# grossmanlev/FL-distributed-delay

Measured on AMD Instinct MI355X. Metric: simulated worker-steps/sec (node) @1024 workers, delay 50; aggregation HBM GB/s, higher is better.
Workload: dtype f32

## Files before the change

### fl-distributed-delay_amd/csrc/gemm_direct.h

```cpp
#pragma once
#include "loaders.h"

namespace flsim {

#ifndef FLSIM_DIRECT_FENCES
#define FLSIM_DIRECT_FENCES 1
#endif
constexpr bool DIRECT_FENCES = FLSIM_DIRECT_FENCES;

template <int IH, int IW, int CI, int PAD, int FM, bool WIN = false, int OHX = 0,
          class SRC = BufSrc>
struct Im2colDirect {
    using Unit = typename SRC::Unit;
    static constexpr int PIX = SRC::SM ? GK : CI;
    static constexpr int SLICE = SRC::SM ? IH * IW * GK : GK;
    static constexpr int OH = OHX > 0 ? OHX : IH + 2 * PAD - 2;
    static constexpr int OW = OHX > 0 ? OHX : IW + 2 * PAD - 2;
    static constexpr int PH = OH / 2, PW = OW / 2;
    static constexpr int ROWS_PER_IMG = WIN ? 4 * PH * PW : OH * OW;
    static_assert(CI % 16 == 0, "direct A needs whole 16-channel slices");

    const float* X;
    const float* XL = nullptr;
    int M;
    unsigned vb[FM];
    unsigned short tapmask[FM];
    SRC buf;

    __device__ void setup(int r0, int lane) {
        const int q = lane >> 4;
        buf.init(X, XL, (unsigned long)((M + ROWS_PER_IMG - 1) / ROWS_PER_IMG) * IH * IW * CI * 4);
#pragma unroll
        for (int f = 0; f < FM; ++f) {
            const int m = r0 + 16 * f + (lane & 15);
            long base = 0;
            int msk = 0;
            if (m < M) {
                const int nimg = m / ROWS_PER_IMG;
                const int rem = m - nimg * ROWS_PER_IMG;
                int oh, ow;
                if constexpr (WIN) {
                    const int qq = rem >> 2;
                    const int ph = qq / PW;
                    oh = 2 * ph + ((rem >> 1) & 1);
                    ow = 2 * (qq - ph * PW) + (rem & 1);
                } else {
                    oh = rem / OW;
                    ow = rem - oh * OW;
                }
                base = (long)nimg * IH * IW * CI + ((long)(oh - PAD) * IW + (ow - PAD)) * PIX +
                       4 * q;
#pragma unroll
                for (int t = 0; t < 9; ++t) {
                    const int ih = oh + t / 3 - PAD, iw = ow + t % 3 - PAD;
                    if ((unsigned)ih < (unsigned)IH && (unsigned)iw < (unsigned)IW) msk |= 1 << t;
                }
            }
            vb[f] = (unsigned)base * 4u;
            tapmask[f] = (unsigned short)msk;
        }
    }
    __device__ void load(int ks, Unit (&r)[FM]) const {
        const int cs = ks / 9;
        const int khkw = ks - 9 * cs;
        const int kh = khkw / 3;
        const unsigned off = (unsigned)(((kh * IW + (khkw - 3 * kh)) * PIX + cs * SLICE) * 4);
#pragma unroll
        for (int f = 0; f < FM; ++f) r[f] = buf.ld_or0(vb[f] + off, (tapmask[f] >> khkw) & 1);
    }
};

template <int TR, int NT>
struct RowsKCStage {
    static constexpr int ROWS = TR;
    static constexpr bool KC = true;
    static constexpr int TOTAL = ROWS * 4;
    static constexpr int UNITS = (TOTAL + NT - 1) / NT;
    static constexpr int FLOATS = KCTile<ROWS>::FLOATS + 4;
    const float* P;
    long ld;
    int NR;
    unsigned rowb[UNITS];
    int dst[UNITS];
    BufSrc buf;
    __device__ void setup(int r0, int tid) {
        buf.init(P, (unsigned long)NR * ld * 4);
#pragma unroll
        for (int j = 0; j < UNITS; ++j) {
            const int u0 = tid + j * NT;
            const bool real = u0 < TOTAL;
            const int u = real ? u0 : u0 % TOTAL;
            const int r = u >> 2, q = u & 3;
            rowb[j] = r0 + r < NR ? (unsigned)(((long)(r0 + r) * ld + 4 * q) * 4) : BUF_OOB;
            dst[j] = real ? KCTile<ROWS>::chunk_off(r, q) : KCTile<ROWS>::FLOATS;
        }
    }
    __device__ void load(int ks, f32x4 (&r)[UNITS]) const {
#pragma unroll
        for (int j = 0; j < UNITS; ++j)
            r[j] = buf.ld(rowb[j] == BUF_OOB ? BUF_OOB : rowb[j] + (unsigned)(ks * GK * 4));
    }
    __device__ void store(float* lds, const f32x4 (&r)[UNITS]) const {
#pragma unroll
        for (int j = 0; j < UNITS; ++j) *reinterpret_cast<f32x4*>(lds + dst[j]) = r[j];
    }
};

template <int FM, int FN, int WAVES, int KB, int DEPTH, class AD, class BL, class EPI>
__global__ void __launch_bounds__(64 * WAVES)
gemm_direct_kernel(AD ad, BL bl, EPI epi, int ksteps, int tiles_m, int tiles_n) {
    constexpr int BM = 16 * FM * WAVES;
    constexpr int BN = 16 * FN;
    static_assert(BL::ROWS == BN && BL::KC, "B loader: k-contiguous tile of BN rows");
    constexpr int BFL = BL::FLOATS;
    constexpr int STG = KB * BFL;
    constexpr bool STAGED = IsStaged<EPI>::value;
    constexpr int STAGE_LD = BN + 4;
    constexpr int BASE_FL = 2 * STG;
    constexpr int WROWS = 16 * FM;
    constexpr int WM_FIT = (BASE_FL > 8192 ? BASE_FL : 8192) / (WROWS * STAGE_LD);
    constexpr int WM_PASS = WM_FIT < 1 ? 1 : (WM_FIT > WAVES ? WAVES : WM_FIT);
    constexpr int LDS_FL = STAGED && WM_PASS * WROWS * STAGE_LD > BASE_FL
                               ? WM_PASS * WROWS * STAGE_LD : BASE_FL;
    __shared__ __attribute__((aligned(16))) float lds[LDS_FL];

    const int tid = threadIdx.x;
    const int lane = tid & 63;
    const int wave = tid >> 6;
    const int nb = gridDim.x;
    const int b = blockIdx.x;
    const int q = nb / 8, r = nb % 8, xcd = b % 8;
    const int L = (xcd < r ? xcd * (q + 1) : r * (q + 1) + (xcd - r) * q) + b / 8;
    const int tn = L % tiles_n;
    const int tm = L / tiles_n;
    const int m0 = tm * BM;
    const int n0 = tn * BN;

    ad.setup(m0 + wave * WROWS, lane);
    bl.setup(n0, tid);

    f32x4 acc[FM][FN];
#pragma unroll
    for (int i = 0; i < FM; ++i)
#pragma unroll
        for (int j = 0; j < FN; ++j) acc[i][j] = f32x4{0.f, 0.f, 0.f, 0.f};

    constexpr int R = DEPTH + 1;
    static_assert(KB % R == 0, "the A register ring index must be static");
    f32x4 ra[R][FM];
    f32x4 rb[BL::UNITS];
    const int nst = ksteps / KB;
#pragma unroll
    for (int d = 0; d < DEPTH; ++d) ad.load(d, ra[d]);
#pragma unroll
    for (int kk = 0; kk < KB; ++kk) {
        bl.load(kk, rb);
        bl.store(lds + kk * BFL, rb);
    }
    __syncthreads();
    if constexpr (WAVES == 8) {
        if (wave >= 4) __builtin_amdgcn_s_setprio(1);
    }
    for (int s = 0; s < nst; ++s) {
        const float* Bs = lds + (s & 1) * STG;
        float* Bn = lds + ((s + 1) & 1) * STG;
        const int kn = (s + 1) * KB;
#pragma unroll
        for (int kk = 0; kk < KB; ++kk) {
            const int ks = s * KB + kk;
            if (kk > 0) bl.store(Bn + (kk - 1) * BFL, rb);
            bl.load(kn + kk, rb);
            ad.load(ks + DEPTH, ra[(kk + DEPTH) % R]);
            if constexpr (DIRECT_FENCES) __builtin_amdgcn_sched_barrier(0);
            f32x4 bf[FN];
#pragma unroll
            for (int j = 0; j < FN; ++j) bf[j] = read_frag<true, BN>(Bs + kk * BFL, 16 * j, lane);
#pragma unroll
            for (int kq = 0; kq < 4; ++kq)
#pragma unroll
                for (int i = 0; i < FM; ++i)
#pragma unroll
                    for (int j = 0; j < FN; ++j)
                        acc[i][j] = mfma16(ra[kk % R][i][kq], bf[j][kq], acc[i][j]);
            if constexpr (DIRECT_FENCES) __builtin_amdgcn_sched_barrier(0);
        }
        bl.store(Bn + (KB - 1) * BFL, rb);
        __syncthreads();
    }

    if constexpr (STAGED) {
        static_assert(BN == EPI::NCOL || (IsPartial<EPI>::value && EPI::NCOL % BN == 0),
                      "staged epilogue needs the full row in one block");
        constexpr int PASSES = (WAVES + WM_PASS - 1) / WM_PASS;
#pragma unroll 1
        for (int pass = 0; pass < PASSES; ++pass) {
            __syncthreads();
            if (wave / WM_PASS == pass) {
#pragma unroll
                for (int i = 0; i < FM; ++i)
#pragma unroll
                    for (int j = 0; j < FN; ++j) {
                        const int ml = (wave - pass * WM_PASS) * WROWS + 16 * i + 4 * (lane >> 4);
                        const int nl = 16 * j + (lane & 15);
#pragma unroll
                        for (int rr = 0; rr < 4; ++rr)
                            lds[(ml + rr) * STAGE_LD + nl] = epi.value(nl, acc[i][j][rr]);
                    }
            }
            __syncthreads();
            const int w_hi = (pass + 1) * WM_PASS < WAVES ? (pass + 1) * WM_PASS : WAVES;
            staged_store(epi, lds, STAGE_LD, m0 + pass * WM_PASS * WROWS,
                         (w_hi - pass * WM_PASS) * WROWS, n0, BN, tid, 64 * WAVES);
        }
    } else {
#pragma unroll
        for (int i = 0; i < FM; ++i)
#pragma unroll
            for (int j = 0; j < FN; ++j) {
                const int m = m0 + wave * WROWS + 16 * i + 4 * (lane >> 4);
                const int n = n0 + 16 * j + (lane & 15);
                epi.apply4(m, n, 0, acc[i][j]);
            }
    }
}
// ... 3 lines not shown
```

### fl-distributed-delay_amd/csrc/gemm_dx6.h

```cpp
#pragma once
#include "gemm_direct.h"
#include "gemm_x6.h"

namespace flsim {

#ifndef FLSIM_DX6_FENCES
#define FLSIM_DX6_FENCES 1
#endif
constexpr bool DX6_FENCES = FLSIM_DX6_FENCES;

template <int TR, int NT, int NPL>
struct RowsKCStageXs {
    using Unit = XsUnit;
    static constexpr int ROWS = TR;
    static constexpr bool KC = true;
    static constexpr int TOTAL = ROWS * 4;
    static constexpr int UNITS = (TOTAL + NT - 1) / NT;
    static constexpr int PLANE = KCTile<ROWS>::FLOATS;
    static constexpr int SPARE = NPL * PLANE;
    static constexpr int FLOATS = NPL * PLANE + 4;
    static_assert(NPL == 2 || NPL == 3, "");
    const float* P;
    const float* PL;
    long ld;
    int NR;
    unsigned rowb[UNITS];
    int dst[UNITS];
    XsSrc buf;
    __device__ void setup(int r0, int tid) {
        buf.init(P, PL, (unsigned long)NR * ld * 4);
#pragma unroll
        for (int j = 0; j < UNITS; ++j) {
            const int u0 = tid + j * NT;
            const bool real = u0 < TOTAL;
            const int u = real ? u0 : u0 % TOTAL;
            const int r = u >> 2, q = u & 3;
            rowb[j] = r0 + r < NR ? (unsigned)(((long)(r0 + r) * ld + 4 * q) * 4) : BUF_OOB;
            dst[j] = real ? KCTile<ROWS>::chunk_off(r, q) : -1;
        }
    }
    __device__ void load(int ks, Unit (&r)[UNITS]) const {
#pragma unroll
        for (int j = 0; j < UNITS; ++j)
            r[j] = buf.ld(rowb[j] == BUF_OOB ? BUF_OOB : rowb[j] + (unsigned)(ks * GK * 4));
    }
    __device__ void store(float* lds, const Unit (&r)[UNITS]) const {
#pragma unroll
        for (int j = 0; j < UNITS; ++j) {
            const bool real = TOTAL % NT == 0 || dst[j] >= 0;
            *reinterpret_cast<f32x4*>(lds + (real ? dst[j] : SPARE)) = r[j].hm;
            *reinterpret_cast<f32x4*>(lds + (real ? dst[j] + PLANE : SPARE)) = xs_lh(r[j]);
            if constexpr (NPL == 3)
                *reinterpret_cast<f32x4*>(lds + (real ? dst[j] + 2 * PLANE : SPARE)) =
                    f32x4{r[j].hm.z, r[j].hm.w, r[j].hm.x, r[j].hm.y};
        }
    }
};

template <int FM, int FN, int WAVES, int KB, int DEPTH, class AD, class BL, class EPI>
__global__ void __launch_bounds__(64 * WAVES)
gemm_dx6_kernel(AD ad, BL bl, EPI epi, int ksteps, int tiles_m, int tiles_n) {
    constexpr int BM = 16 * FM * WAVES;
    constexpr int BN = 16 * FN;
    static_assert(BL::ROWS == BN && BL::KC, "B loader: k-contiguous tile of BN rows");
    constexpr int BFL = BL::FLOATS;
    constexpr int PLANE = BL::PLANE;
    constexpr int STG = KB * BFL;
    constexpr bool STAGED = IsStaged<EPI>::value;
    constexpr int STAGE_LD = BN + 4;
    constexpr int BASE_FL = 2 * STG;
    constexpr int WROWS = 16 * FM;
    constexpr int WM_FIT = (BASE_FL > 8192 ? BASE_FL : 8192) / (WROWS * STAGE_LD);
    constexpr int WM_PASS = WM_FIT < 1 ? 1 : (WM_FIT > WAVES ? WAVES : WM_FIT);
    constexpr int LDS_FL = STAGED && WM_PASS * WROWS * STAGE_LD > BASE_FL
                               ? WM_PASS * WROWS * STAGE_LD : BASE_FL;
    static_assert(LDS_FL * 4 <= 160 * 1024, "LDS");
    __shared__ __attribute__((aligned(16))) float lds[LDS_FL];

    const int tid = threadIdx.x;
    const int lane = tid & 63;
    const int wave = tid >> 6;
    const int nb = gridDim.x;
    const int b = blockIdx.x;
    const int q = nb / 8, r = nb % 8, xcd = b % 8;
    const int L = (xcd < r ? xcd * (q + 1) : r * (q + 1) + (xcd - r) * q) + b / 8;
    const int tn = L % tiles_n;
    const int tm = L / tiles_n;
    const int m0 = tm * BM;
    const int n0 = tn * BN;

    ad.setup(m0 + wave * WROWS, lane);
    bl.setup(n0, tid);

    f32x4 acc[FM][FN];
#pragma unroll
    for (int i = 0; i < FM; ++i)
#pragma unroll
        for (int j = 0; j < FN; ++j) acc[i][j] = f32x4{0.f, 0.f, 0.f, 0.f};

    constexpr int R = DEPTH + 1;
    static_assert(KB % R == 0, "the A register ring index must be static");
    XsUnit ra[R][FM];
    typename BL::Unit rb[BL::UNITS];
    const int nst = ksteps / KB;
#pragma unroll
    for (int d = 0; d < DEPTH; ++d) ad.load(d, ra[d]);
#pragma unroll
    for (int kk = 0; kk < KB; ++kk) {
        bl.load(kk, rb);
        bl.store(lds + kk * BFL, rb);
    }
    __syncthreads();
    if constexpr (WAVES == 8) {
        if (wave >= 4) __builtin_amdgcn_s_setprio(1);
    }
    for (int s = 0; s < nst; ++s) {
        const float* Bs = lds + (s & 1) * STG;
        float* Bn = lds + ((s + 1) & 1) * STG;
        const int kn = (s + 1) * KB;
#pragma unroll
        for (int kk = 0; kk < KB; ++kk) {
            const int ks = s * KB + kk;
            if (kk > 0) bl.store(Bn + (kk - 1) * BFL, rb);
            bl.load(kn + kk, rb);
            ad.load(ks + DEPTH, ra[(kk + DEPTH) % R]);
            if constexpr (DX6_FENCES) __builtin_amdgcn_sched_barrier(0);
            const float* Bk = Bs + kk * BFL;
            f32x4 a0[FM], a1[FM];
#pragma unroll
            for (int i = 0; i < FM; ++i) {
                a0[i] = ra[kk % R][i].hm;
                a1[i] = xs_hl(ra[kk % R][i]);
            }
#pragma unroll
            for (int j = 0; j < FN; ++j) {
                const f32x4 x0 = read_frag<true, BN>(Bk, 16 * j, lane);
                const f32x4 x2 = read_frag<true, BN>(Bk + PLANE, 16 * j, lane);
                f32x4 x1;
                if constexpr (BFL >= 3 * PLANE)
                    x1 = read_frag<true, BN>(Bk + 2 * PLANE, 16 * j, lane);
                else
                    x1 = f32x4{x0.z, x0.w, x0.x, x0.y};
#pragma unroll
                for (int i = 0; i < FM; ++i) {
                    acc[i][j] = x6_step<x6_fresh(true)>(acc[i][j], a0[i], a1[i], x0, x1, x2);
                }
            }
            if constexpr (DX6_FENCES) __builtin_amdgcn_sched_barrier(0);
        }
        bl.store(Bn + (KB - 1) * BFL, rb);
        __syncthreads();
    }

    if constexpr (STAGED) {
        static_assert(BN == EPI::NCOL || (IsPartial<EPI>::value && EPI::NCOL % BN == 0),
                      "staged epilogue needs the full row in one block");
        constexpr int PASSES = (WAVES + WM_PASS - 1) / WM_PASS;
#pragma unroll 1
        for (int pass = 0; pass < PASSES; ++pass) {
            __syncthreads();
            if (wave / WM_PASS == pass) {
#pragma unroll
                for (int i = 0; i < FM; ++i)
#pragma unroll
                    for (int j = 0; j < FN; ++j) {
                        const int ml = (wave - pass * WM_PASS) * WROWS + 16 * i + 4 * (lane >> 4);
                        const int nl = 16 * j + (lane & 15);
#pragma unroll
                        for (int rr = 0; rr < 4; ++rr)
                            lds[(ml + rr) * STAGE_LD + nl] = epi.value(nl, acc[i][j][rr]);
                    }
            }
            __syncthreads();
            const int w_hi = (pass + 1) * WM_PASS < WAVES ? (pass + 1) * WM_PASS : WAVES;
            staged_store(epi, lds, STAGE_LD, m0 + pass * WM_PASS * WROWS,
                         (w_hi - pass * WM_PASS) * WROWS, n0, BN, tid, 64 * WAVES);
        }
    } else {
#pragma unroll
        for (int i = 0; i < FM; ++i)
#pragma unroll
            for (int j = 0; j < FN; ++j) {
                const int m = m0 + wave * WROWS + 16 * i + 4 * (lane >> 4);
                const int n = n0 + 16 * j + (lane & 15);
                epi.apply4(m, n, 0, acc[i][j]);
            }
    }
}

}
```

### fl-distributed-delay_amd/csrc/net_kernels.h

```cpp
#pragma once
#include "epi_xs.h"
#include "gemm_direct.h"
#include "gemm_dx6.h"
#include "gemm_x6.h"
#include "loaders.h"
#include "pn1.h"
#include "probe.h"

namespace flsim {

static __global__ void __launch_bounds__(256)
k_fill_batch(const uint8_t* __restrict__ pool, const int32_t* __restrict__ labels,
             const int32_t* __restrict__ list_a, int len_a, const int32_t* __restrict__ list_b,
             int len_b, const WorkerRec* __restrict__ workers, int n_workers_total, uint64_t seed,
             const float* __restrict__ lut, float* __restrict__ x0, int32_t* __restrict__ y) {
    const int s = blockIdx.x;
    const int w = s / SAMPLES_PER_WORKER;
    const int j = s - w * SAMPLES_PER_WORKER;
    const WorkerRec wr = workers[w];
    const uint32_t bsz = wr.pad ? wr.pad : (uint32_t)SAMPLES_PER_WORKER;
    const uint32_t q = (wr.i >> 20) * SAMPLES_PER_WORKER + (uint32_t)j;
    float* out = x0 + (long)s * 4096;
    if (q >= bsz) {
        if (threadIdx.x == 0) y[s] = -1;
// ... 690 lines not shown
    }
    if (kmin <= 0) return Z;
    int z = (ksteps + kmin - 1) / kmin;
    const int zb = (1024 + tiles - 1) / tiles;
    if (z < zb) z = zb;
    static int fill = -1;
    if (fill < 0) {
        const char* e = lab_env("FLSIM_WSPLIT_FILL");
        fill = e ? atoi(e) : 0;
    }
    if (fill && cap > 0 && z < Z) {
        const long rounds = ((long)tiles * z + cap - 1) / cap;
        const long zf = rounds * cap / tiles;
        if (zf > z) z = (int)(zf < ksteps ? zf : ksteps);
    }
    return z < Z ? z : Z;
}

static int resident_blocks(const void* f, int nt) {
    static int cus = 0;
    if (!cus) {
        int dev = 0;
        if (hipGetDevice(&dev) != hipSuccess ||
            hipDeviceGetAttribute(&cus, hipDeviceAttributeMultiprocessorCount, dev) != hipSuccess)
            cus = -1;
    }
    int per = 0;
    if (cus <= 0 || hipOccupancyMaxActiveBlocksPerMultiprocessor(&per, f, nt, 0) != hipSuccess)
        return 0;
    return per * cus;
}

template <int IH, int IW, int CI, int PAD, int FM, int FN, int WM, int WN, class EPI, int OHX = 0,
          bool X6 = false>
static int conv_like(const float* X, int S, const float* Wpk, int N, int KP, const EPI& epi,
                     hipStream_t st, int kid, int kreal) {
    constexpr int NT = 64 * WM * WN;
    constexpr int BM = 16 * FM * WM, BN = 16 * FN * WN;
    using AL = Im2colKC<IH, IW, CI, PAD, BM, NT, false, OHX>;
    using BL = RowsKC<BN, NT>;
    AL al;
    al.X = X;
    al.M = S * AL::OH * AL::OW;
    BL bl;
    bl.P = Wpk;
    bl.ld = KP;
    bl.NR = N;
    return launch_gemm<FM, FN, WM, WN, X6>(al, bl, epi, al.M, N, KP / GK, 1, st, kid,
                                           2.0 * al.M * N * kreal);
}

template <int IH, int IW, int CI, int PAD, int FM, int FN, int WM, int WN, int OHX = 0, class EPI>
static int conv_x6(const float* X, int S, const float* Wpk, int N, int KP, const EPI& epi,
                   hipStream_t st, int kid, int kreal) {
    return conv_like<IH, IW, CI, PAD, FM, FN, WM, WN, EPI, OHX, true>(X, S, Wpk, N, KP, epi, st,
                                                                      kid, kreal);
}

template <int IH, int IW, int CI, int PAD, int FM, int FMS, int FN, int WM, int WN, class EPI>
static int conv_like_sz(const float* X, int S, const float* Wpk, int N, int KP, const EPI& epi,
                        hipStream_t st, int kid, int kreal) {
    if (S <= small_chunk_samples())
        return conv_like<IH, IW, CI, PAD, FMS, FN, WM, WN>(X, S, Wpk, N, KP, epi, st, kid, kreal);
    return conv_like<IH, IW, CI, PAD, FM, FN, WM, WN>(X, S, Wpk, N, KP, epi, st, kid, kreal);
}

template <int IH, int IW, int CI, int PAD, int FM, int FN, int WM, int WN, int VO = 0,
          bool DZC = false, bool X6 = false, class SRC = BufSrc, class SRCB = SRC>
static int conv_wgrad(const float* dz, const float* X, int S, int CO, int KP, float* slab,
                      float* bslab, int Z, hipStream_t st, int kid, int kreal,
                      int zinit = 0x7fffffff, int* zused = nullptr, const float* dzl = nullptr,
                      const float* Xl = nullptr) {
    constexpr int NT = 64 * WM * WN;
    constexpr int BM = 16 * FM * WM, BN = 16 * FN * WN;
    constexpr int OFULL = IH + 2 * PAD - 2;
    static_assert(IH == IW && VO <= OFULL, "square maps only");
    static_assert(X6 || (!SRC::SPLIT && !SRCB::SPLIT), "split operands run on the split-bf16 GEMM");
    using AL = RowsKM<BM, NT, (VO > 0 && !DZC ? OFULL : 0), (DZC ? 0 : VO), SRC>;
    using BL = Im2colKM<IH, IW, CI, PAD, BN, NT, VO, SRCB>;
    const int M = S * BL::OH * BL::OW;
    AL al;
    al.P = dz;
    al.PL = dzl;
    al.ld = CO;
    al.NK = M;
    al.NC = CO;
    BL bl;
    bl.X = X;
    bl.XL = Xl;
    bl.M = M;
    EpiSlabAcc epi{slab, CO, KP, (long)CO * KP, bslab, zinit};
    const int tiles = ceil_div(CO, BM) * ceil_div(KP, BN);
    const void* kfn;
    if constexpr (X6)
        kfn = (const void*)gemm_x6_kernel<FM, FN, WM, WN, AL, BL, EpiSlabAcc>;
    else
        kfn = (const void*)gemm_kernel<FM, FN, WM, WN, AL, BL, EpiSlabAcc>;
    static const int cap = resident_blocks(kfn, NT);
    const int zu = wsplit(ceil_div(M, GK), Z, tiles, cap);
    if (zused) *zused = zu;
    return launch_gemm<FM, FN, WM, WN, X6>(al, bl, epi, CO, KP, ceil_div(M, GK), zu, st, kid,
                                           2.0 * M * CO * kreal);
}

template <int IH, int IW, int CI, int FM, int FN, int WM, int WN, int DH, class SRCB = BufSrc>
static int conv_wgrad_dense(const float* dz, const float* X, int S, int CO, int KP, float* slab,
                            float* bslab, int Z, hipStream_t st, int kid, int kreal,
                            int zinit = 0x7fffffff, int* zused = nullptr) {
    constexpr int NT = 64 * WM * WN;
    constexpr int BM = 16 * FM * WM, BN = 16 * FN * WN;
    static_assert(IH == IW, "square maps only");
    static_assert(BN == CI, "an n-tile is exactly one filter tap");
    using AL = TapRowsKM<IH, IW, CI, DH, BM, NT>;
    using BL = PixRowsKM<IH, IW, CI, BN, NT, SRCB>;
    FLSIM_REQUIRE(KP == 9 * CI, "dense weight gradient: %d columns, not 9 taps of %d", KP, CI);
    const int M = S * IH * IW;
    AL al;
    al.P = dz;
    al.ld = CO;
    al.M = M;
    al.NC = CO;
    BL bl;
    bl.X = X;
    bl.M = M;
    EpiSlabAccRing epi{{slab, CO, KP, (long)CO * KP, bslab, zinit}};
    const int tm = ceil_div(CO, BM), tn = KP / BN;
    static const int cap =
        resident_blocks((const void*)gemm_kernel<FM, FN, WM, WN, AL, BL, EpiSlabAccRing>, NT);
    const int ksteps = ceil_div(M, GK);
    const int zu = wsplit(ksteps, Z, tm * tn, cap);
    if (zused) *zused = zu;
    const int per = (ksteps + zu - 1) / zu;
    const ProbeSlot ps = probe_begin();
    hipExtLaunchKernelGGL((gemm_kernel<FM, FN, WM, WN, AL, BL, EpiSlabAccRing>), dim3(tm * tn * zu),
                          dim3(NT), 0, st, ps.start, ps.stop, 0, al, bl, epi, ksteps, per, tm, tn);
    FLSIM_LAUNCH_CHECK();
    return probe_end(ps, kid, 2.0 * M * CO * kreal);
}

template <int IH, int IW, int CI, int PAD, int FM, int FN, int WM, int WN, int FMS, int FNS,
          int WMS, int WNS, int VO = 0, bool DZC = false, bool X6 = false, class SRC = BufSrc,
          class SRCB = SRC>
static int conv_wgrad_sz(const float* dz, const float* X, int S, int CO, int KP, float* slab,
                         float* bslab, int Z, hipStream_t st, int kid, int kreal, int zinit,
                         int* zused, const float* dzl = nullptr, const float* Xl = nullptr) {
    if (S <= small_chunk_samples())
        return conv_wgrad<IH, IW, CI, PAD, FMS, FNS, WMS, WNS, VO, DZC, X6, SRC, SRCB>(
            dz, X, S, CO, KP, slab, bslab, Z, st, kid, kreal, zinit, zused, dzl, Xl);
    return conv_wgrad<IH, IW, CI, PAD, FM, FN, WM, WN, VO, DZC, X6, SRC, SRCB>(
        dz, X, S, CO, KP, slab, bslab, Z, st, kid, kreal, zinit, zused, dzl, Xl);
}

template <int IH, int IW, int CI, int PAD, int FM, int FN, int WAVES, int KB, int DEPTH, int NPL,
          bool WIN, int OHX, class ASRC = XsSrc, class EPI>
static int conv_dx6(XsT X, int S, XsT W, int N, int KP, const EPI& epi, hipStream_t st, int kid,
                    int kreal) {
    static_assert(ASRC::SPLIT, "split input");
    using AD = Im2colDirect<IH, IW, CI, PAD, FM, WIN, OHX, ASRC>;
    using BL = RowsKCStageXs<16 * FN, 64 * WAVES, NPL>;
    constexpr int BM = 16 * FM * WAVES, BN = 16 * FN;
    FLSIM_REQUIRE((KP / GK) % KB == 0, "direct GEMM: %d k-steps not a multiple of %d", KP / GK, KB);
    AD ad;
    ad.X = X.hm;
    ad.XL = X.l;
    ad.M = S * AD::ROWS_PER_IMG;
    BL bl;
    bl.P = W.hm;
    bl.PL = W.l;
    bl.ld = KP;
    bl.NR = N;
    const int tm = ceil_div(ad.M, BM), tn = ceil_div(N, BN);
    const ProbeSlot ps = probe_begin();
    hipExtLaunchKernelGGL((gemm_dx6_kernel<FM, FN, WAVES, KB, DEPTH, AD, BL, EPI>),
                          dim3(tm * tn), dim3(64 * WAVES), 0, st, ps.start, ps.stop, 0, ad, bl,
                          epi, KP / GK, tm, tn);
    FLSIM_LAUNCH_CHECK();
    return probe_end(ps, kid, 2.0 * ad.M * N * kreal);
}

template <int IH, int IW, int CI, int PAD, int FM, int FN, int WM, int WN, bool WIN, int OHX,
          class EPI>
static int conv_xs(XsT X, int S, XsT W, int N, int KP, const EPI& epi, hipStream_t st, int kid,
                   int kreal) {
    constexpr int NT = 64 * WM * WN;
    constexpr int BM = 16 * FM * WM, BN = 16 * FN * WN;
    using AL = Im2colKC<IH, IW, CI, PAD, BM, NT, WIN, OHX, XsSrc>;
    using BL = RowsKC<BN, NT, XsSrc>;
    AL al;
    al.X = X.hm;
    al.XL = X.l;
    al.M = S * AL::ROWS_PER_IMG;
    BL bl;
    bl.P = W.hm;
    bl.PL = W.l;
    bl.ld = KP;
    bl.NR = N;
    return launch_gemm<FM, FN, WM, WN, true>(al, bl, epi, al.M, N, KP / GK, 1, st, kid,
                                             2.0 * al.M * N * kreal);
}

template <int IH, int IW, int CI, int CO, int PAD, int FM, int FN, int WM, int WN, bool NCHW_OUT,
          bool X6 = false>
static int conv_pool_fwd(const float* X, int S, const float* Wpk, int KP, float* d, uint8_t* idx,
                         const float* bias, const WorkerRec* workers, uint64_t seed, uint32_t site,
                         uint32_t thr, float scale, int dropout, hipStream_t st, int kid,
                         int kreal) {
    constexpr int NT = 64 * WM * WN;
    constexpr int BM = 16 * FM * WM, BN = 16 * FN * WN;
    using AL = Im2colKC<IH, IW, CI, PAD, BM, NT, true>;
    using BL = RowsKC<BN, NT>;
    AL al;
    al.X = X;
    al.M = S * AL::ROWS_PER_IMG;
    BL bl;
    bl.P = Wpk;
    bl.ld = KP;
    bl.NR = CO;
    EpiPoolDrop<AL::PH, AL::PW, CO, NCHW_OUT> epi{d, idx, bias, workers, seed, site, thr,
                                                  scale, dropout, al.M};
    return launch_gemm<FM, FN, WM, WN, X6>(al, bl, epi, al.M, CO, KP / GK, 1, st, kid,
                                           2.0 * al.M * CO * kreal);
}

template <int FM, int FN, int WM, int WN, bool X6 = false, class EPI = EpiSlabStore>
static int linear_fwd(const float* x, const float* W, float* part, int M, int N, int K, int Z,
                      hipStream_t st, int kid) {
    constexpr int NT = 64 * WM * WN;
    RowsKC<16 * FM * WM, NT> al{};
    al.P = x; al.ld = K; al.NR = M;
    RowsKC<16 * FN * WN, NT> bl{};
    bl.P = W; bl.ld = K; bl.NR = N;
    EPI epi{};
    static_cast<EpiSlabStore&>(epi) = EpiSlabStore{part, M, N, (long)M * N};
    return launch_gemm<FM, FN, WM, WN, X6>(al, bl, epi, M, N, K / GK, Z, st, kid, 2.0 * M * N * K);
}

template <int FM, int FN, int WM, int WN, bool X6 = false>
static int linear_wgrad(const float* dy, const float* x, float* slab, float* bslab, int S, int N,
                        int K, int Z, hipStream_t st, int kid, int zinit = 0x7fffffff,
                        int* zused = nullptr) {
    constexpr int NT = 64 * WM * WN;
    RowsKM<16 * FM * WM, NT> al{};
    al.P = dy; al.ld = N; al.NK = S; al.NC = N;
    RowsKM<16 * FN * WN, NT> bl{};
    bl.P = x; bl.ld = K; bl.NK = S; bl.NC = K;
    EpiSlabAcc epi{slab, N, K, (long)N * K, bslab, zinit};
    const int tiles = ceil_div(N, 16 * FM * WM) * ceil_div(K, 16 * FN * WN);
    const int zu = wsplit(ceil_div(S, GK), Z, tiles);
    if (zused) *zused = zu;
    return launch_gemm<FM, FN, WM, WN, X6>(al, bl, epi, N, K, ceil_div(S, GK), zu, st, kid,
                                           2.0 * S * N * K);
}

template <int FM, int FN, int WM, int WN, bool X6 = false>
static int linear_dgrad(const float* dy, const float* W, float* dx, const float* act, float scale,
                        int S, int N, int K, hipStream_t st, int kid) {
    constexpr int NT = 64 * WM * WN;
    RowsKC<16 * FM * WM, NT> dl{};
    dl.P = dy; dl.ld = N; dl.NR = S;
    RowsKM<16 * FN * WN, NT> wl{};
    wl.P = W; wl.ld = K; wl.NK = N; wl.NC = K;
    EpiDropMaskPre de{{dx, act, scale, S, K}};
    return launch_gemm<FM, FN, WM, WN, X6>(dl, wl, de, S, K, N / GK, 1, st, kid,
                                           2.0 * S * N * K);
}

}
```

### fl-distributed-delay_amd/csrc/pn1_net.hip

```cpp
#include <stdarg.h>
#include <stdio.h>
#include <string.h>

#include <mutex>
#include <unordered_map>

#include "net_abi.h"

namespace flsim {

static thread_local char g_err[512];
void set_error(const char* fmt, ...) {
    va_list ap;
    va_start(ap, fmt);
    vsnprintf(g_err, sizeof(g_err), fmt, ap);
    va_end(ap);
}
const char* last_error() { return g_err; }

struct ConvGeo {
    int CI, CIP, CO, H;
    int KP;
    int ZW;
};
// ... 93 lines not shown
    return g;
}

struct WS {
    float* x0; float* a1; float* a2; float* d1; float* a3; float* a4; float* d2; float* a5;
    float* a6; float* d3; float* e1; float* e2; float* part; float* dh1; float* dh2;
    float* gx; float* gy; float* loss_s; float* dlog; int32_t* y;
    uint8_t* i1; uint8_t* i2; uint8_t* i3;
    float* a1l; float* d1l; float* a3l; float* d2l; float* a5l;
    float* a6l; float* a4l; float* a2l; float* gxl;
    float* a1f; float* d1f; float* a3f; float* d2f; float* a5f;
    long bytes;
    XsT x(float* hm, float* l) const { return XsT{hm, l}; }
};

static WS ws_layout(char* base, int S, int row0 = 0) {
    WS w;
    long o = 0;
    auto take_rows = [&](long per_bytes) {
        char* p = base ? base + o + per_bytes * row0 : nullptr;
        o += (per_bytes * S + 255) / 256 * 256;
        return p;
    };
    auto tf = [&](long per) { return (float*)take_rows(per * 4); };
    w.x0 = tf(4096); w.a1 = tf(55488); w.a2 = tf(62208); w.d1 = tf(15552);
    w.a3 = tf(38400); w.a4 = tf(46464); w.d2 = tf(11616); w.a5 = tf(32448);
    w.a6 = tf(43200); w.d3 = tf(9408); w.e1 = tf(512); w.e2 = tf(256);
    w.part = tf(512L * ZL1F); w.dh1 = tf(512); w.dh2 = tf(256);
    w.gx = tf(55488); w.gy = tf(15552); w.loss_s = tf(1); w.dlog = tf(16);
    w.y = (int32_t*)take_rows(4);
    w.i1 = (uint8_t*)take_rows(15552); w.i2 = (uint8_t*)take_rows(11616);
    w.i3 = (uint8_t*)take_rows(9408);
    w.a1l = tf(55488 / 2); w.d1l = tf(15552 / 2); w.a3l = tf(38400 / 2); w.d2l = tf(11616 / 2);
    w.a5l = tf(32448 / 2);
    w.a6l = tf(0); w.a4l = tf(0); w.a2l = tf(0); w.gxl = tf(0);
    w.a1f = tf(55488); w.d1f = tf(15552); w.a3f = tf(38400); w.d2f = tf(11616); w.a5f = tf(32448);
    w.bytes = o;
    return w;
}

static int pack_weights(const GradState& g, const float* theta, hipStream_t st) {
    RC(pack_conv(theta + P_OFF[0], g.wf[0], nullptr, GEO[0].CO, GEO[0].CI, GEO[0].CIP, GEO[0].KP,
                 st));
    for (int l = 1; l < 6; ++l) {
        const ConvGeo& c = GEO[l];
        RC(pack_conv_xs(theta + P_OFF[2 * l], g.wfx[l], g.wdx[l], c.CO, c.CI, c.KP, st));
        hipLaunchKernelGGL(k_pack_dgrad, dim3(ceil_div((long)c.CI * 9 * c.CO, 256)), dim3(256), 0,
                           st, theta + P_OFF[2 * l], g.wd[l], c.CO, c.CI);
        FLSIM_LAUNCH_CHECK();
    }
    return 0;
}

constexpr int C1_ROWS = 32;
static_assert(C1_ROWS == 32, "the a1 store loop maps 64 lanes to 16 rows x 4 units of a slice");
constexpr int C1_LD = 52;
__global__ void __launch_bounds__(256)
k_conv1_fwd(const float* __restrict__ x0, const float* __restrict__ W, const float* __restrict__ bias,
            float* __restrict__ a1, float* __restrict__ a1l, float* __restrict__ a1f, long units) {
    __shared__ __attribute__((aligned(16))) float stage[4][C1_ROWS * C1_LD];
    const int lane = threadIdx.x & 63, wv = threadIdx.x >> 6;
    const int i = lane & 15, g = lane >> 4;
    float* st = stage[wv];
    f32x4 wb[3][2];
    float w8[3], bj[3];
#pragma unroll
    for (int j = 0; j < 3; ++j) {
        const int co = 16 * j + i;
#pragma unroll
        for (int sx = 0; sx < 2; ++sx) {
            const int tap = 4 * sx + g;
            wb[j][sx] = f32x4{W[(co * 3 + 0) * 9 + tap], W[(co * 3 + 1) * 9 + tap],
                              W[(co * 3 + 2) * 9 + tap], 0.f};
        }
        w8[j] = g < 3 ? W[(co * 3 + g) * 9 + 8] : 0.f;
        bj[j] = bias[co];
    }
    BufSrc xb;
    xb.init(x0, (unsigned long)(units * C1_ROWS / 1156) * 4096 * 4);
    auto load = [&](long u, f32x4 (&xa)[2][2], float (&x8)[2]) {
#pragma unroll
        for (int t = 0; t < 2; ++t) {
            const unsigned m = (unsigned)u * C1_ROWS + 16 * t + i;
            const unsigned smp = m / 1156u;
            const int rem = (int)(m - smp * 1156u);
            const int oh = rem / 34, ow = rem - (rem / 34) * 34;
            const unsigned xs = smp * 4096u;
#pragma unroll
            for (int sx = 0; sx < 2; ++sx) {
                const int tap = 4 * sx + g;
                const int ih = oh + tap / 3 - 2, iw = ow + tap % 3 - 2;
                xa[t][sx] = xb.ld_or0((xs + (unsigned)(ih * 32 + iw) * 4u) * 4u,
                                      (unsigned)ih < 32u && (unsigned)iw < 32u);
            }
            x8[t] = (oh < 32 && ow < 32) ? x0[xs + (oh * 32 + ow) * 4 + g] : 0.f;
        }
    };
    const long nw = (long)gridDim.x * 4;
    long u = (long)blockIdx.x * 4 + wv;
    f32x4 xa[2][2];
    float x8[2];
    if (u < units) load(u, xa, x8);
    for (; u < units; u += nw) {
        f32x4 acc[2][3];
#pragma unroll
        for (int t = 0; t < 2; ++t)
#pragma unroll
            for (int j = 0; j < 3; ++j) {
                f32x4 c = zero4();
#pragma unroll
                for (int sx = 0; sx < 2; ++sx)
#pragma unroll
                    for (int kk = 0; kk < 4; ++kk) c = mfma16(xa[t][sx][kk], wb[j][sx][kk], c);
                acc[t][j] = mfma16(x8[t], w8[j], c);
            }
        if (u + nw < units) load(u + nw, xa, x8);
#pragma unroll
        for (int t = 0; t < 2; ++t)
#pragma unroll
            for (int j = 0; j < 3; ++j)
#pragma unroll
                for (int r = 0; r < 4; ++r)
                    st[(16 * t + 4 * g + r) * C1_LD + 16 * j + i] = fmaxf(acc[t][j][r] + bj[j], 0.f);
        __builtin_amdgcn_wave_barrier();
#pragma unroll
        for (int q0 = 0; q0 < C1_ROWS * 12; q0 += 64) {
            const int q = q0 + lane, slice = q >> 7, row = (q & 127) >> 2, c4 = 4 * slice + (q & 3);
            xs_store_f(a1, a1l, a1f, xs_unit<48, 1156, true>((unsigned)(u * C1_ROWS + row), c4),
                       *reinterpret_cast<const f32x4*>(st + row * C1_LD + 4 * c4));
        }
        __builtin_amdgcn_wave_barrier();
    }
}

static int conv1_fwd(const float* x0, const float* W, const float* bias, XsT a1, float* a1f,
                     int S, hipStream_t st) {
    const long M = (long)S * 34 * 34;
    if (M % C1_ROWS) return 1;
    const long units = M / C1_ROWS;
    const int grid = (int)(units / 4 < 2048 ? (units + 3) / 4 : 2048);
    const ProbeSlot ps = probe_begin();
    hipExtLaunchKernelGGL(k_conv1_fwd, dim3(grid), dim3(256), 0, st, ps.start, ps.stop, 0, x0, W,
                          bias, a1.hm, a1.l, a1f, units);
    FLSIM_LAUNCH_CHECK();
    return probe_end(ps, K_FWD1, 2.0 * M * 48 * 27);
}

#ifndef FLSIM_DX_FM
#define FLSIM_DX_FM 4
#endif
constexpr int DX_FM = FLSIM_DX_FM, DX_FMS = 1, DX_KB = 3, DX_DEPTH = 2, DX_NPL = 2;


template <int IH, int IW, int CI, int PAD, int FN, bool WIN, int OHX, int FM = DX_FM,
          int WAVES = 8, int FMS = (FM == DX_FM ? DX_FMS : FM / 2), class EPI>
static int dx6(XsT X, int S, XsT W, int N, int KP, const EPI& epi, hipStream_t st, int kid,
               int kreal) {
    if (S <= small_chunk_samples())
        return conv_dx6<IH, IW, CI, PAD, FMS, FN, WAVES, DX_KB, DX_DEPTH, DX_NPL, WIN, OHX,
                        XsSrcSM>(X, S, W, N, KP, epi, st, kid, kreal);
    return conv_dx6<IH, IW, CI, PAD, FM, FN, WAVES, DX_KB, DX_DEPTH, DX_NPL, WIN, OHX, XsSrcSM>(
        X, S, W, N, KP, epi, st, kid, kreal);
}

template <int IH, int IW, int CI, int PAD, int FM, int FN, int WM, int WN, bool WIN, int OHX,
          class EPI>
static int xs(XsT X, int S, XsT W, int N, int KP, const EPI& epi, hipStream_t st, int kid,
              int kreal) {
    if (S <= small_chunk_samples())
        return conv_xs<IH, IW, CI, PAD, FM / 2, FN, WM, WN, WIN, OHX>(X, S, W, N, KP, epi, st, kid,
                                                                     kreal);
    return conv_xs<IH, IW, CI, PAD, FM, FN, WM, WN, WIN, OHX>(X, S, W, N, KP, epi, st, kid, kreal);
}

static int forward(const GradState& g, const WS& w, const float* theta, int S,
                   const WorkerRec* workers, uint64_t seed, int dropout, hipStream_t st) {
    const XsT a1 = w.x(w.a1, w.a1l), d1 = w.x(w.d1, w.d1l), a3 = w.x(w.a3, w.a3l);
    const XsT d2 = w.x(w.d2, w.d2l), a5 = w.x(w.a5, w.a5l);
    RC(conv1_fwd(w.x0, theta + P_OFF[0], theta + P_OFF[1], a1, w.a1f, S, st));
    RC((dx6<34, 34, 48, 2, 3, true, 0, 4, 4, 2>(a1, S, g.wfx[1], 48, 432,
        EpiPoolDropXs<18, 18, 48, true>{d1.hm, d1.l, w.i1, theta + P_OFF[3], workers, seed, SITE_DROP1,
                                  THR_P25, SCALE_P25, dropout, S * 18 * 18 * 4, w.d1f}, st,
        K_FWD2, 432)));
    RC((dx6<18, 18, 48, 2, 6, false, 0>(d1, S, g.wfx[2], 96, 432,
        EpiBiasReluXs<96, true, 400>{a3.hm, a3.l, theta + P_OFF[5], S * 20 * 20, w.a3f}, st, K_FWD3,
        432)));
    RC((dx6<20, 20, 96, 2, 6, true, 0>(a3, S, g.wfx[3], 96, 864,
        EpiPoolDropXs<11, 11, 96>{d2.hm, d2.l, w.i2, theta + P_OFF[7], workers, seed, SITE_DROP2,
                                  THR_P25, SCALE_P25, dropout, S * 11 * 11 * 4, w.d2f}, st,
        K_FWD4, 864)));
    RC((xs<11, 11, 96, 2, 4, 6, 4, 2, false, 0>(d2, S, g.wfx[4], 192, 864,
        EpiBiasReluXs<192>{a5.hm, a5.l, theta + P_OFF[9], S * 13 * 13, w.a5f}, st, K_FWD5, 864)));
    RC((xs<13, 13, 192, 2, 4, 6, 4, 2, true, 0>(a5, S, g.wfx[5], 192, 1728,
        EpiPoolDrop<7, 7, 192, true>{w.d3, w.i3, theta + P_OFF[11], workers, seed, SITE_DROP3,
                                     THR_P25, SCALE_P25, dropout, S * 7 * 7 * 4}, st, K_FWD6,
        1728)));
    if (S <= 2048)
        RC((linear_fwd<1, 2, 2, 2, true, EpiSlabStoreFresh>(w.d3, theta + P_OFF[12], w.part, S,
                                                            512, 9408, ZL1F, st, K_L1F)));
    else if (S <= 4096)
        RC((linear_fwd<2, 2, 2, 2, true, EpiSlabStoreFresh>(w.d3, theta + P_OFF[12], w.part, S,
                                                            512, 9408, ZL1F, st, K_L1F)));
    else
        RC((linear_fwd<4, 4, 2, 2, true, EpiSlabStoreFresh>(w.d3, theta + P_OFF[12], w.part, S,
                                                            512, 9408, ZL1F, st, K_L1F)));
    RC(linear_finish(w.part, ZL1F, theta + P_OFF[13], w.e1, S, 512, workers, seed, SITE_DROP4,
                     THR_P50, SCALE_P50, dropout, st));
    RC((linear_fwd<2, 2, 2, 2>(w.e1, theta + P_OFF[14], w.part, S, 256, 512, 1, st, K_L2F)));
    RC(linear_finish(w.part, 1, theta + P_OFF[15], w.e2, S, 256, workers, seed, SITE_DROP5,
                     THR_P50, SCALE_P50, dropout, st));
    return 0;
}

struct EpochRows {
    int z[8];
};

struct Pipe {
    hipStream_t bs = nullptr;
    hipEvent_t fwd_done = nullptr, bwd_tail = nullptr;
    std::unordered_map<const void*, hipEvent_t> ws_free;
    bool pending = false;
};

struct HostState {
    EpochRows rows{};
    Pipe pipe;
};
static std::mutex g_state_mu;
static std::unordered_map<const void*, HostState> g_state;

static HostState* find_state(const void* gradstate) {
    auto it = g_state.find(gradstate);
    return it == g_state.end() ? nullptr : &it->second;
}


static int pipe_join(const void* gradstate, hipStream_t st) {
    std::lock_guard<std::mutex> lk(g_state_mu);
    HostState* hs = find_state(gradstate);
    if (!hs || !hs->pipe.pending) return 0;
    Pipe& p = hs->pipe;
    FLSIM_CHECK_HIP(hipEventRecord(p.bwd_tail, p.bs));
    FLSIM_CHECK_HIP(hipStreamWaitEvent(st, p.bwd_tail, 0));
    p.pending = false;
    return 0;
}

static int wait_workspace(const Pipe& p, const void* workspace, hipStream_t stream) {
    auto e = p.ws_free.find(workspace);
    if (e != p.ws_free.end() && e->second)
        FLSIM_CHECK_HIP(hipStreamWaitEvent(stream, e->second, 0));
    return 0;
}

static int begin_rows(const void* gradstate, const void* workspace, bool need_epoch,
                      hipStream_t stream) {
    std::lock_guard<std::mutex> lk(g_state_mu);
    const HostState* hs = find_state(gradstate);
    FLSIM_REQUIRE(hs || !need_epoch, "forward rows without flsim_pn1_begin_epoch");
    return hs ? wait_workspace(hs->pipe, workspace, stream) : 0;
}

static StepPlan plan_in_use(const GradState& g, const void* gradstate) {
    EpochRows er;
    {
        std::lock_guard<std::mutex> lk(g_state_mu);
        const HostState* hs = find_state(gradstate);
        if (!hs) return g.plan;
        er = hs->rows;
    }
    SegSpec specs[STEP_MAX_SEG];
    const int n = pn1_segments(g, reinterpret_cast<const float*>(gradstate), specs);
    int zin[STEP_MAX_SEG];
    for (int i = 0; i < n; ++i) {
        zin[i] = specs[i].Z;
        if (specs[i].group >= 0) {
            const int z = er.z[specs[i].group];
            zin[i] = z < specs[i].Z ? z : specs[i].Z;
            specs[i].Z = zin[i] > 0 ? zin[i] : 1;
        }
    }
    StepPlan p;
    plan_step(specs, n, &p);
    for (int i = 0; i < p.nseg; ++i)
        for (int j = 0; j < n; ++j)
            if (specs[j].slab_off == p.seg[i].slab_off) p.seg[i].zlim = zin[j];
    return p;
}

struct SideStream {
    hipStream_t s = nullptr;
    hipEvent_t to_side = nullptr, to_main = nullptr;
    std::mutex* mu = nullptr;
};
static SideStream* side_stream() {
    static std::mutex mu;
    static std::unordered_map<int, SideStream> per_dev;
    int dev = 0;
    if (hipGetDevice(&dev) != hipSuccess) return nullptr;
    std::lock_guard<std::mutex> lk(mu);
    SideStream& ss = per_dev[dev];
    if (!ss.s) {
        if (hipStreamCreateWithFlags(&ss.s, hipStreamNonBlocking) != hipSuccess ||
            hipEventCreateWithFlags(&ss.to_side, hipEventDisableTiming) != hipSuccess ||
            hipEventCreateWithFlags(&ss.to_main, hipEventDisableTiming) != hipSuccess) {
            ss = SideStream{};
            return nullptr;
        }
        ss.mu = new std::mutex();
    }
    return &ss;
}
static bool concurrent_backward(int S) {
    static int smax = -1;
    if (smax < 0) {
        const char* e = lab_env("FLSIM_CONCURRENT_BWD");
        smax = e ? atoi(e) : 2048;
    }
    return S <= smax;
}

#ifndef FLSIM_DG_FMS
#define FLSIM_DG_FMS 2
#endif
constexpr int DG_FMS = FLSIM_DG_FMS;

#ifndef FLSIM_WGRAD_X6
#define FLSIM_WGRAD_X6 0
#endif

#ifndef FLSIM_WGD2
#define FLSIM_WGD2 0
#endif
#ifndef FLSIM_WGD3
#define FLSIM_WGD3 1
#endif
#ifndef FLSIM_WGD4
#define FLSIM_WGD4 1
#endif
// ... 422 lines not shown
```

Before: 1161.

## Share im2col tap loads between neighbouring output pixels in forward conv GEMMs

Adds an im2col A-loader that assigns neighbouring output pixels to consecutive MFMA fragments, so one filter row (kh) needs only FM+2 global loads instead of 3*FM. Each stage loads one filter row's units and reuses them across the three kw taps. The main loop is restructured with a two-slot register ring, and the staged epilogue un-permutes the rows. It is enabled by default for forward conv layers 2-4 on the large-chunk path. The cost is more registers held across the ring and a requirement for a staged epilogue.

After: 1169, median of 6. Within noise of the previous version (+0.7%).

```diff
diff --git a/fl-distributed-delay_amd/csrc/gemm_direct.h b/fl-distributed-delay_amd/csrc/gemm_direct.h
--- a/fl-distributed-delay_amd/csrc/gemm_direct.h
+++ b/fl-distributed-delay_amd/csrc/gemm_direct.h
@@ -70,6 +70,142 @@
     }
 };
 
+template <int FM, bool WIN>
+struct TapShareRows {
+    static constexpr int ROWS = 16 * FM;
+    static constexpr int row(int f, int r) {
+        if (!WIN) return FM * r + f;
+        const int x = FM * (r >> 1) + f, y = r & 1;
+        return 4 * (x >> 1) + 2 * y + (x & 1);
+    }
+    static constexpr int strip_x(int l) { return WIN ? 2 * (l >> 2) + (l & 1) : l; }
+    static constexpr int frag(int l) { return strip_x(l) % FM; }
+    static constexpr int mrow(int l) {
+        return WIN ? 2 * (strip_x(l) / FM) + ((l >> 1) & 1) : l / FM;
+    }
+    static constexpr bool bijection() {
+        for (int l = 0; l < ROWS; ++l)
+            if (frag(l) < 0 || frag(l) >= FM || mrow(l) < 0 || mrow(l) >= 16 ||
+                row(frag(l), mrow(l)) != l)
+                return false;
+        for (int f = 0; f < FM; ++f)
+            for (int r = 0; r < 16; ++r)
+                if (row(f, r) < 0 || row(f, r) >= ROWS || frag(row(f, r)) != f ||
+                    mrow(row(f, r)) != r)
+                    return false;
+        return true;
+    }
+    static constexpr int next(int m) { return WIN && (m & 1) ? m + 3 : m + 1; }
+    static constexpr bool neighbours() {
+        for (int f = 0; f + 1 < FM; ++f)
+            for (int r = 0; r < 16; ++r)
+                if (row(f + 1, r) != next(row(f, r))) return false;
+        return true;
+    }
+};
+
+template <int IH, int IW, int CI, int PAD, bool WIN, bool SM>
+struct TapShareGeo {
+    static constexpr int PIX = SM ? GK : CI;
+    static constexpr int SLICE = SM ? IH * IW * GK : GK;
+    static constexpr int OH = IH + 2 * PAD - 2;
+    static constexpr int OW = IW + 2 * PAD - 2;
+    static constexpr int PH = OH / 2, PW = OW / 2;
+    static constexpr int ROWS_PER_IMG = WIN ? 4 * PH * PW : OH * OW;
+    struct Pix {
+        int nimg, oh, ow;
+    };
+    static constexpr Pix pixel(int m) {
+        const int nimg = m / ROWS_PER_IMG;
+        const int rem = m - nimg * ROWS_PER_IMG;
+        if (WIN) {
+            const int qq = rem >> 2;
+            const int ph = qq / PW;
+            return Pix{nimg, 2 * ph + ((rem >> 1) & 1), 2 * (qq - ph * PW) + (rem & 1)};
+        }
+        return Pix{nimg, rem / OW, rem % OW};
+    }
+    static constexpr bool tap_ok(const Pix& p, int kh, int kw) {
+        return (unsigned)(p.oh + kh - PAD) < (unsigned)IH &&
+               (unsigned)(p.ow + kw - PAD) < (unsigned)IW;
+    }
+    static constexpr long tap_off(const Pix& p, int kh, int kw) {
+        return (long)p.nimg * IH * IW * CI +
+               ((long)(p.oh + kh - PAD) * IW + (p.ow + kw - PAD)) * PIX;
+    }
+    static constexpr int next(int m) { return TapShareRows<1, WIN>::next(m); }
+    static constexpr bool shares(int kh) {
+        for (int m = 0; m < ROWS_PER_IMG; ++m) {
+            const Pix p = pixel(m), n = pixel(next(m));
+            for (int kw = 0; kw < 2; ++kw) {
+                const bool a = tap_ok(p, kh, kw + 1), b = tap_ok(n, kh, kw);
+                if (a != b || (a && tap_off(p, kh, kw + 1) != tap_off(n, kh, kw))) return false;
+            }
+        }
+        return true;
+    }
+};
+
+template <int IH, int IW, int CI, int PAD, int FM, bool WIN = false, int OHX = 0,
+          class SRC = XsSrc>
+struct Im2colDirectShare : TapShareGeo<IH, IW, CI, PAD, WIN, SRC::SM> {
+    static constexpr bool SHARE_TAPS = true;
+    using Unit = typename SRC::Unit;
+    using Rows = TapShareRows<FM, WIN>;
+    using Geo = TapShareGeo<IH, IW, CI, PAD, WIN, SRC::SM>;
+    using Pix = typename Geo::Pix;
+    using Geo::PIX, Geo::SLICE, Geo::OH, Geo::OW, Geo::ROWS_PER_IMG;
+    using Geo::pixel, Geo::tap_ok, Geo::tap_off;
+    static constexpr int NJ = FM + 2;
+    static_assert(SRC::SPLIT, "split sources");
+    static_assert(CI % 16 == 0, "direct A needs whole 16-channel slices");
+    static_assert(PAD == 2 && OHX == 0 && OW == IW + 2, "tap sharing needs the padded width IW + 2");
+    static_assert(!WIN || (OW % 2 == 0 && OH % 2 == 0), "whole pool windows");
+    static_assert(Rows::bijection(), "row assignment");
+    static_assert(Rows::neighbours(), "fragment f + 1 holds fragment f's next rows");
+    static_assert(Geo::shares(0) && Geo::shares(1) && Geo::shares(2),
+                  "neighbouring pixels share their taps");
+
+    const float* X;
+    const float* XL = nullptr;
+    int M;
+    unsigned vb[FM];
+    unsigned short tapmask[FM];
+    SRC buf;
+
+    __device__ void setup(int r0, int lane) {
+        const int q = lane >> 4;
+        buf.init(X, XL, (unsigned long)((M + ROWS_PER_IMG - 1) / ROWS_PER_IMG) * IH * IW * CI * 4);
+#pragma unroll
+        for (int f = 0; f < FM; ++f) {
+            const int m = r0 + Rows::row(f, lane & 15);
+            long base = 0;
+            int msk = 0;
+            if (m < M) {
+                const Pix p = pixel(m);
+                base = tap_off(p, 0, 0) + 4 * q;
+#pragma unroll
+                for (int t = 0; t < 9; ++t)
+                    if (tap_ok(p, t / 3, t % 3)) msk |= 1 << t;
+            }
+            vb[f] = (unsigned)base * 4u;
+            tapmask[f] = (unsigned short)msk;
+        }
+    }
+    __device__ Unit load(int row, int t) const {
+        const int cs = row / 3;
+        const int kh = row - 3 * cs;
+        const int f = t < FM ? t : FM - 1, kw = t < FM ? 0 : t - FM + 1;
+        const unsigned off = (unsigned)(((kh * IW + kw) * PIX + cs * SLICE) * 4);
+        return buf.ld_or0(vb[f] + off, (tapmask[f] >> (3 * kh + kw)) & 1);
+    }
+};
+
+template <class AD, class = void>
+struct SharesTaps : std::false_type {};
+template <class AD>
+struct SharesTaps<AD, std::void_t<decltype(AD::SHARE_TAPS)>> : std::bool_constant<AD::SHARE_TAPS> {};
+
 template <int TR, int NT>
 struct RowsKCStage {
     static constexpr int ROWS = TR;
diff --git a/fl-distributed-delay_amd/csrc/gemm_dx6.h b/fl-distributed-delay_amd/csrc/gemm_dx6.h
--- a/fl-distributed-delay_amd/csrc/gemm_dx6.h
+++ b/fl-distributed-delay_amd/csrc/gemm_dx6.h
@@ -98,13 +98,24 @@
 #pragma unroll
         for (int j = 0; j < FN; ++j) acc[i][j] = f32x4{0.f, 0.f, 0.f, 0.f};
 
-    constexpr int R = DEPTH + 1;
-    static_assert(KB % R == 0, "the A register ring index must be static");
-    XsUnit ra[R][FM];
+    constexpr bool SHARE = SharesTaps<AD>::value;
+    static_assert(!SHARE || (KB == 3 && DEPTH == 2 && STAGED),
+                  "shared taps: one filter row per stage, rows permuted in the staging tile");
+    constexpr int R = SHARE ? 2 : DEPTH + 1;
+    constexpr int NA = SHARE ? FM + 2 : FM;
+    constexpr int NJK = (NA + KB - 1) / KB;
+    constexpr int SP = SHARE ? 2 : 1;
+    static_assert(SHARE || KB % R == 0, "the A register ring index must be static");
+    XsUnit ra[R][NA];
     typename BL::Unit rb[BL::UNITS];
     const int nst = ksteps / KB;
-#pragma unroll
-    for (int d = 0; d < DEPTH; ++d) ad.load(d, ra[d]);
+    if constexpr (SHARE) {
+#pragma unroll
+        for (int t = 0; t < NA; ++t) ra[0][t] = ad.load(0, t);
+    } else {
+#pragma unroll
+        for (int d = 0; d < DEPTH; ++d) ad.load(d, ra[d]);
+    }
 #pragma unroll
     for (int kk = 0; kk < KB; ++kk) {
         bl.load(kk, rb);
@@ -114,42 +125,55 @@
     if constexpr (WAVES == 8) {
         if (wave >= 4) __builtin_amdgcn_s_setprio(1);
     }
-    for (int s = 0; s < nst; ++s) {
-        const float* Bs = lds + (s & 1) * STG;
-        float* Bn = lds + ((s + 1) & 1) * STG;
-        const int kn = (s + 1) * KB;
-#pragma unroll
-        for (int kk = 0; kk < KB; ++kk) {
-            const int ks = s * KB + kk;
-            if (kk > 0) bl.store(Bn + (kk - 1) * BFL, rb);
-            bl.load(kn + kk, rb);
-            ad.load(ks + DEPTH, ra[(kk + DEPTH) % R]);
-            if constexpr (DX6_FENCES) __builtin_amdgcn_sched_barrier(0);
-            const float* Bk = Bs + kk * BFL;
-            f32x4 a0[FM], a1[FM];
-#pragma unroll
-            for (int i = 0; i < FM; ++i) {
-                a0[i] = ra[kk % R][i].hm;
-                a1[i] = xs_hl(ra[kk % R][i]);
+    for (int s0 = 0; s0 < nst; s0 += SP) {
+#pragma unroll
+        for (int sp = 0; sp < SP; ++sp) {
+            const int s = s0 + sp;
+            if (SP > 1 && s >= nst) break;
+            const int par = SHARE ? sp : s & 1;
+            const float* Bs = lds + par * STG;
+            float* Bn = lds + (par ^ 1) * STG;
+            const int kn = (s + 1) * KB;
+#pragma unroll
+            for (int kk = 0; kk < KB; ++kk) {
+                const int ks = s * KB + kk;
+                if (kk > 0) bl.store(Bn + (kk - 1) * BFL, rb);
+                bl.load(kn + kk, rb);
+                if constexpr (SHARE) {
+#pragma unroll
+                    for (int t = NJK * kk; t < NJK * (kk + 1) && t < NA; ++t)
+                        ra[sp ^ 1][t] = ad.load(s + 1, t);
+                } else {
+                    ad.load(ks + DEPTH, ra[(kk + DEPTH) % R]);
+                }
+                if constexpr (DX6_FENCES) __builtin_amdgcn_sched_barrier(0);
+                const float* Bk = Bs + kk * BFL;
+                f32x4 a0[FM], a1[FM];
+#pragma unroll
+                for (int i = 0; i < FM; ++i) {
+                    const XsUnit& u = ra[SHARE ? sp : kk % R][SHARE ? i + kk : i];
+                    a0[i] = u.hm;
+                    a1[i] = xs_hl(u);
+                }
+#pragma unroll
+                for (int j = 0; j < FN; ++j) {
+                    const f32x4 x0 = read_frag<true, BN>(Bk, 16 * j, lane);
+                    const f32x4 x2 = read_frag<true, BN>(Bk + PLANE, 16 * j, lane);
+                    f32x4 x1;
+                    if constexpr (BFL >= 3 * PLANE)
+                        x1 = read_frag<true, BN>(Bk + 2 * PLANE, 16 * j, lane);
+                    else
+                        x1 = f32x4{x0.z, x0.w, x0.x, x0.y};
+#pragma unroll
+                    for (int i = 0; i < FM; ++i) {
+                        acc[i][j] = x6_step<x6_fresh(true)>(acc[i][j], a0[i], a1[i], x0, x1, x2);
+                    }
+                }
+                if constexpr (DX6_FENCES) __builtin_amdgcn_sched_barrier(0);
             }
-#pragma unroll
-            for (int j = 0; j < FN; ++j) {
-                const f32x4 x0 = read_frag<true, BN>(Bk, 16 * j, lane);
-                const f32x4 x2 = read_frag<true, BN>(Bk + PLANE, 16 * j, lane);
-                f32x4 x1;
-                if constexpr (BFL >= 3 * PLANE)
-                    x1 = read_frag<true, BN>(Bk + 2 * PLANE, 16 * j, lane);
-                else
-                    x1 = f32x4{x0.z, x0.w, x0.x, x0.y};
-#pragma unroll
-                for (int i = 0; i < FM; ++i) {
-                    acc[i][j] = x6_step<x6_fresh(true)>(acc[i][j], a0[i], a1[i], x0, x1, x2);
-                }
-            }
-            if constexpr (DX6_FENCES) __builtin_amdgcn_sched_barrier(0);
-        }
-        bl.store(Bn + (KB - 1) * BFL, rb);
-        __syncthreads();
+            bl.store(Bn + (KB - 1) * BFL, rb);
+            __syncthreads();
+        }
     }
 
     if constexpr (STAGED) {
@@ -164,11 +188,14 @@
                 for (int i = 0; i < FM; ++i)
 #pragma unroll
                     for (int j = 0; j < FN; ++j) {
-                        const int ml = (wave - pass * WM_PASS) * WROWS + 16 * i + 4 * (lane >> 4);
+                        const int mw = (wave - pass * WM_PASS) * WROWS;
                         const int nl = 16 * j + (lane & 15);
 #pragma unroll
-                        for (int rr = 0; rr < 4; ++rr)
-                            lds[(ml + rr) * STAGE_LD + nl] = epi.value(nl, acc[i][j][rr]);
+                        for (int rr = 0; rr < 4; ++rr) {
+                            int ml = 16 * i + 4 * (lane >> 4) + rr;
+                            if constexpr (SHARE) ml = AD::Rows::row(i, 4 * (lane >> 4) + rr);
+                            lds[(mw + ml) * STAGE_LD + nl] = epi.value(nl, acc[i][j][rr]);
+                        }
                     }
             }
             __syncthreads();
@@ -177,6 +204,7 @@
                          (w_hi - pass * WM_PASS) * WROWS, n0, BN, tid, 64 * WAVES);
         }
     } else {
+        static_assert(!SHARE, "the shared-tap row order needs a staged epilogue");
 #pragma unroll
         for (int i = 0; i < FM; ++i)
 #pragma unroll
diff --git a/fl-distributed-delay_amd/csrc/net_kernels.h b/fl-distributed-delay_amd/csrc/net_kernels.h
--- a/fl-distributed-delay_amd/csrc/net_kernels.h
+++ b/fl-distributed-delay_amd/csrc/net_kernels.h
@@ -866,11 +866,12 @@
 }
 
 template <int IH, int IW, int CI, int PAD, int FM, int FN, int WAVES, int KB, int DEPTH, int NPL,
-          bool WIN, int OHX, class ASRC = XsSrc, class EPI>
+          bool WIN, int OHX, class ASRC = XsSrc, bool SHARE = false, class EPI>
 static int conv_dx6(XsT X, int S, XsT W, int N, int KP, const EPI& epi, hipStream_t st, int kid,
                     int kreal) {
     static_assert(ASRC::SPLIT, "split input");
-    using AD = Im2colDirect<IH, IW, CI, PAD, FM, WIN, OHX, ASRC>;
+    using AD = std::conditional_t<SHARE, Im2colDirectShare<IH, IW, CI, PAD, FM, WIN, OHX, ASRC>,
+                                  Im2colDirect<IH, IW, CI, PAD, FM, WIN, OHX, ASRC>>;
     using BL = RowsKCStageXs<16 * FN, 64 * WAVES, NPL>;
     constexpr int BM = 16 * FM * WAVES, BN = 16 * FN;
     FLSIM_REQUIRE((KP / GK) % KB == 0, "direct GEMM: %d k-steps not a multiple of %d", KP / GK, KB);
diff --git a/fl-distributed-delay_amd/csrc/pn1_net.hip b/fl-distributed-delay_amd/csrc/pn1_net.hip
--- a/fl-distributed-delay_amd/csrc/pn1_net.hip
+++ b/fl-distributed-delay_amd/csrc/pn1_net.hip
@@ -269,15 +269,25 @@
 constexpr int DX_FM = FLSIM_DX_FM, DX_FMS = 1, DX_KB = 3, DX_DEPTH = 2, DX_NPL = 2;
 
 
-template <int IH, int IW, int CI, int PAD, int FN, bool WIN, int OHX, int FM = DX_FM,
+#ifndef FLSIM_FWS2
+#define FLSIM_FWS2 1
+#endif
+#ifndef FLSIM_FWS3
+#define FLSIM_FWS3 1
+#endif
+#ifndef FLSIM_FWS4
+#define FLSIM_FWS4 1
+#endif
+
+template <int IH, int IW, int CI, int PAD, int FN, bool WIN, int OHX, bool SHARE, int FM = DX_FM,
           int WAVES = 8, int FMS = (FM == DX_FM ? DX_FMS : FM / 2), class EPI>
 static int dx6(XsT X, int S, XsT W, int N, int KP, const EPI& epi, hipStream_t st, int kid,
                int kreal) {
     if (S <= small_chunk_samples())
         return conv_dx6<IH, IW, CI, PAD, FMS, FN, WAVES, DX_KB, DX_DEPTH, DX_NPL, WIN, OHX,
                         XsSrcSM>(X, S, W, N, KP, epi, st, kid, kreal);
-    return conv_dx6<IH, IW, CI, PAD, FM, FN, WAVES, DX_KB, DX_DEPTH, DX_NPL, WIN, OHX, XsSrcSM>(
-        X, S, W, N, KP, epi, st, kid, kreal);
+    return conv_dx6<IH, IW, CI, PAD, FM, FN, WAVES, DX_KB, DX_DEPTH, DX_NPL, WIN, OHX, XsSrcSM,
+                    SHARE>(X, S, W, N, KP, epi, st, kid, kreal);
 }
 
 template <int IH, int IW, int CI, int PAD, int FM, int FN, int WM, int WN, bool WIN, int OHX,
@@ -295,14 +305,14 @@
     const XsT a1 = w.x(w.a1, w.a1l), d1 = w.x(w.d1, w.d1l), a3 = w.x(w.a3, w.a3l);
     const XsT d2 = w.x(w.d2, w.d2l), a5 = w.x(w.a5, w.a5l);
     RC(conv1_fwd(w.x0, theta + P_OFF[0], theta + P_OFF[1], a1, w.a1f, S, st));
-    RC((dx6<34, 34, 48, 2, 3, true, 0, 4, 4, 2>(a1, S, g.wfx[1], 48, 432,
+    RC((dx6<34, 34, 48, 2, 3, true, 0, FLSIM_FWS2, 4, 4, 2>(a1, S, g.wfx[1], 48, 432,
         EpiPoolDropXs<18, 18, 48, true>{d1.hm, d1.l, w.i1, theta + P_OFF[3], workers, seed, SITE_DROP1,
                                   THR_P25, SCALE_P25, dropout, S * 18 * 18 * 4, w.d1f}, st,
         K_FWD2, 432)));
-    RC((dx6<18, 18, 48, 2, 6, false, 0>(d1, S, g.wfx[2], 96, 432,
+    RC((dx6<18, 18, 48, 2, 6, false, 0, FLSIM_FWS3>(d1, S, g.wfx[2], 96, 432,
         EpiBiasReluXs<96, true, 400>{a3.hm, a3.l, theta + P_OFF[5], S * 20 * 20, w.a3f}, st, K_FWD3,
         432)));
-    RC((dx6<20, 20, 96, 2, 6, true, 0>(a3, S, g.wfx[3], 96, 864,
+    RC((dx6<20, 20, 96, 2, 6, true, 0, FLSIM_FWS4>(a3, S, g.wfx[3], 96, 864,
         EpiPoolDropXs<11, 11, 96>{d2.hm, d2.l, w.i2, theta + P_OFF[7], workers, seed, SITE_DROP2,
                                   THR_P25, SCALE_P25, dropout, S * 11 * 11 * 4, w.d2f}, st,
         K_FWD4, 864)));
```
